# WangWen-Believer/DR-SLAM

Measured on AMD Instinct MI355X. Metric: RGB-D frames/sec (extract+match) at 640x480, higher is better.
Workload: dtype u8; 1 GPU; 640x480 synthetic RGB-D (TUM3 intrinsics), ORB extract 1000/1.2/8/20/7 + SearchByProjection(frame k, frame k-1, th=15) on consecutive frames; BASELINE config 2; batch_per_gpu=512, batches_in_flight_per_gpu=3, distinct_resident_input_batches_per_gpu=3, sequence_frames_per_rank=64

## Files before the change

dr_slam_amd/csrc/capi_match.cpp:

```cpp
#include "drfe_internal.h"
#include "match_internal.h"
#include "stage_layout.h"
#include "../../include/drfe_math.h"

#include <algorithm>
#include <cmath>
#include <cstdlib>
#include <cstring>
#include <new>
#include <thread>

template <class T>
static hipError_t dalloc(T** p, size_t n)
{
    *p = nullptr;
    return hipMalloc((void**)p, std::max<size_t>(n, 1) * sizeof(T));
}

void drfe_match_buffers_free(drfe_ctx* c)
{
    MatchBuffers* m = c->mb;
    if (!m) return;
    void* ptrs[] = {m->d_pairs, m->d_queries, m->d_mps, m->d_scale, m->d_candIdx, m->d_candKey, m->d_candCnt, m->d_candBest,
                    m->d_hist, m->d_initObs, m->d_bfIdx, m->d_bfDist, m->d_bfQ, m->d_bfT};
// ... 305 lines not shown
{
    if (!c || !offsets || slot < 0 || slot >= c->lastBatch || !c->glueValid) return c ? DRFE_ERR_STATE : DRFE_ERR_INVALID;
    int rc = drfe_stream_sync(c);
    if (rc != DRFE_OK) return rc;
    HIPCHK(c, hipMemcpy(offsets, c->d_gridOff + (size_t)slot * (DRFE_GRID_CELLS + 1), sizeof(int) * (DRFE_GRID_CELLS + 1),
                        hipMemcpyDeviceToHost));
    const int n = offsets[DRFE_GRID_CELLS];
    if (n > cap) return DRFE_ERR_CAPACITY;
    if (n && indices) HIPCHK(c, hipMemcpy(indices, c->d_gridIdx + (size_t)slot * c->maxKp, sizeof(int) * n, hipMemcpyDeviceToHost));
    return DRFE_OK;
}

}

int drfe_match_consecutive_stage(drfe_ctx* c, const float* Tcw, const float* Twc, const drfe_camera* cam, int mono, int nframes, hipStream_t s)
{
    MatchBuffers* m = drfe_match_buffers(c);
    if (!m) return DRFE_ERR_HIP;
    const int np = nframes - 1;
    const size_t pairBytes = sizeof(MatchPair) * (size_t)c->cfg.max_batch, poseBytes = sizeof(float) * 16 * (size_t)c->cfg.max_batch;
    if (!m->h_stage[0]) {
        m->stageBytes = pairBytes + poseBytes;
        for (int k = 0; k < 2; k++) {
            HIPCHK(c, hipHostMalloc(&m->h_stage[k], m->stageBytes, hipHostMallocDefault));
            HIPCHK(c, hipEventCreateWithFlags(&m->stageEv[k], hipEventDisableTiming));
            HIPCHK(c, hipEventRecord(m->stageEv[k], s));
        }
    }
    const int slotK = m->stageNext;
    m->stageNext ^= 1;
    HIPCHK(c, hipEventSynchronize(m->stageEv[slotK]));
    MatchPair* pairs = static_cast<MatchPair*>(m->h_stage[slotK]);
    float* poses = reinterpret_cast<float*>(static_cast<uint8_t*>(m->h_stage[slotK]) + pairBytes);
    std::memcpy(poses, Twc, sizeof(float) * 16 * (size_t)nframes);
    const float mb = cam->bf / cam->fx;
    for (int p = 0; p < np; p++) {
        MatchPair& P = pairs[p];
        P.curSlot = p + 1; P.lastSlot = p; P.mpSlot = p; P.nQueries = 0;
        P.queryBase = p * c->maxKp;
        P.mpBase = p * c->maxKp;
        std::memcpy(P.Tcw, Tcw + (size_t)(p + 1) * 16, sizeof(float) * 16);
        drfe_motion_flags(Tcw + (size_t)(p + 1) * 16, Tcw + (size_t)p * 16, mb, mono, &P.forward, &P.backward);
    }
    HIPCHK(c, hipMemcpyAsync(m->d_pairs, pairs, sizeof(MatchPair) * np, hipMemcpyHostToDevice, s));
    HIPCHK(c, hipMemcpyAsync(c->d_poses, poses, sizeof(float) * 16 * nframes, hipMemcpyHostToDevice, s));
    HIPCHK(c, hipEventRecord(m->stageEv[slotK], s));
    return DRFE_OK;
}

hipError_t drfe_match_consecutive_enqueue(drfe_ctx* c, const drfe_camera* cam, float th, int check_ori, int nframes, hipStream_t s)
{
    MatchBuffers* m = drfe_match_buffers(c);
    if (!m) return hipErrorOutOfMemory;
    hipError_t e = hipMemsetAsync(c->d_match, 0xFF, sizeof(int) * (size_t)nframes * c->maxKp, s);
    if (e == hipSuccess) e = hipMemsetAsync(c->d_matchCount, 0, sizeof(int) * nframes, s);
    if (e == hipSuccess) e = drfe_launch_mappoints_last(c, *m, *cam, c->d_poses, nframes, s);
    if (e == hipSuccess) e = drfe_launch_window_match(c, *m, *cam, nframes - 1, c->maxKp, 0, th, 0.f, check_ori, nullptr, s, 2);
    return e;
}

extern "C" {

int drfe_match_consecutive_batch(drfe_ctx* c, const float* Tcw, const float* Twc, const drfe_camera* cam, float th,
                                 int mono, int check_ori, int nframes, void* stream)
{
    if (!c || !Tcw || !Twc || !cam) return DRFE_ERR_INVALID;
    if (nframes < 2 || nframes > c->lastBatch || !c->glueValid) {
        c->err = "match: needs an extracted batch of >= 2 frames with stereo/grid computed";
        return DRFE_ERR_STATE;
    }
    if (c->maxKp > DRFE_MATCH_LAST_MAX_QUERIES) {
        c->err = "match: the slot size (drfe_orb_max_keypoints = " + std::to_string(c->maxKp) +
                 ") exceeds the 4096 map points the consecutive matcher resolves per pair";
        return DRFE_ERR_CAPACITY;
    }
    HIPCHK(c, hipSetDevice(c->device));
    hipStream_t s = stream ? (hipStream_t)stream : c->stream;
    const int rc = drfe_match_consecutive_stage(c, Tcw, Twc, cam, mono, nframes, s);
    if (rc != DRFE_OK) return rc;
    if (c->profile) { (void)hipEventRecord(c->ev[DRFE_STAGE_MATCH][0], s); c->evUsed[DRFE_STAGE_MATCH] = true; }
    HIPCHK(c, drfe_match_consecutive_enqueue(c, cam, th, check_ori, nframes, s));
    if (c->profile) (void)hipEventRecord(c->ev[DRFE_STAGE_MATCH][1], s);
    return DRFE_OK;
}

int drfe_match_download(drfe_ctx* c, int slot, int32_t* cur_to_last, int cap, int* nmatches)
{
    if (!c || slot < 0 || slot >= c->lastBatch) return c ? DRFE_ERR_STATE : DRFE_ERR_INVALID;
    int rc = drfe_stream_sync(c);
    if (rc != DRFE_OK) return rc;
    rc = match_status(c, 2);
    if (rc != DRFE_OK) return rc;
    int n = 0;
    HIPCHK(c, hipMemcpy(&n, c->d_kpCount + slot, sizeof(int), hipMemcpyDeviceToHost));
    if (n > cap) return DRFE_ERR_CAPACITY;
    if (n && cur_to_last)
        HIPCHK(c, hipMemcpy(cur_to_last, c->d_match + (size_t)slot * c->maxKp, sizeof(int) * n, hipMemcpyDeviceToHost));
    if (nmatches) HIPCHK(c, hipMemcpy(nmatches, c->d_matchCount + slot, sizeof(int), hipMemcpyDeviceToHost));
    return DRFE_OK;
}

int drfe_search_by_projection_last(drfe_ctx* c, int cur_slot, int last_slot, const float* Tcw_cur, const float* Tcw_last,
                                   const drfe_camera* cam, const drfe_map_point* last_mp, int n_last, float th, int mono,
                                   int check_ori, const uint8_t* cur_obs, int32_t* cur_mp, int n_cur, int* nmatches)
{
    if (!c || !Tcw_cur || !Tcw_last || !cam || !last_mp || !cur_mp || !nmatches) return DRFE_ERR_INVALID;
    if (cur_slot < 0 || cur_slot >= c->lastBatch || last_slot < 0 || last_slot >= c->lastBatch || !c->glueValid) {
        c->err = "search_by_projection_last: slots not ready";
        return DRFE_ERR_STATE;
    }
    HIPCHK(c, hipSetDevice(c->device));
// ... 854 lines not shown
```

dr_slam_amd/csrc/match_internal.h:

```cpp
#ifndef DRFE_MATCH_INTERNAL_H
#define DRFE_MATCH_INTERNAL_H
#include "drfe_internal.h"

#define DRFE_MATCH_LAST_MAX_QUERIES 4096

struct MatchPair {
    int curSlot, lastSlot;
    int mpSlot;
    int nQueries;
    int queryBase;
    int mpBase;
    int forward, backward;
    float Tcw[16];
};

struct MatchQuery {
    float u, v, radius;
    float ur, thrR;
    int minLevel, maxLevel;
    int valid;
    int obs;
    uint32_t desc[8];
};

struct MatchBuffers {
    MatchPair* d_pairs = nullptr;
    MatchQuery* d_queries = nullptr;
    drfe_map_point* d_mps = nullptr;
    float* d_scale = nullptr;
    uint32_t* d_candIdx = nullptr;
    uint32_t* d_candKey = nullptr;
    int* d_candCnt = nullptr;
    uint2* d_candBest = nullptr;
    uint16_t* d_hist = nullptr;
    uint8_t* d_initObs = nullptr;
    int32_t* d_bfIdx = nullptr; int32_t* d_bfDist = nullptr; uint8_t* d_bfQ = nullptr; uint8_t* d_bfT = nullptr; size_t bfCap = 0;
    size_t queryCap = 0;
    void* h_stage[2] = {nullptr, nullptr}; hipEvent_t stageEv[2] = {nullptr, nullptr}; size_t stageBytes = 0; int stageNext = 0;
};

hipError_t drfe_launch_window_match(drfe_ctx* c, const MatchBuffers& mb, const drfe_camera& cam, int npairs,
                                    int maxQueries, int mode, float th, float nnratio, int checkOri,
                                    const uint8_t* d_initObs, hipStream_t s, int statusWord = 1);
hipError_t drfe_launch_fill_i32(int* d_p, int n, int v, hipStream_t s);
hipError_t drfe_launch_fill_i32_and_word(int* d_p, int n, int v, int* d_q, int w, hipStream_t s);
struct DrfePackArgs { const uint32_t* src[10]; uint32_t dwords[10]; int n; };
hipError_t drfe_launch_pack_segments(const DrfePackArgs& A, uint32_t* d_dst, hipStream_t s);
void drfe_motion_flags(const float* TcwCur, const float* TcwLast, float mb, int mono, int* fwd, int* bwd);
hipError_t drfe_launch_window_candidates(drfe_ctx* c, const MatchBuffers& mb, const drfe_camera& cam, int npairs, int maxQueries,
                                         hipStream_t s);
hipError_t drfe_launch_mappoints_last(drfe_ctx* c, const MatchBuffers& mb, const drfe_camera& cam, const float* d_Twc,
                                      int nframes, hipStream_t s);
hipError_t drfe_launch_bf_knn(const uint8_t* dQ, int nq, const uint8_t* dT, int nt, int k, int* dIdx, int* dDist,
                              hipStream_t s);

struct LineQuery {
    int valid, obs;
    int minLevel, maxLevel;
    float x1, y1, x2, y2, r;
    uint32_t desc[8];
};
struct LineCur { float ptX, ptY, angle; int octave; };

hipError_t drfe_launch_line_projection(const drfe_map_line* d_lines, int n, const float* d_TcwCur, const drfe_camera& cam,
                                       int forward, int backward, const float* d_scale, float th, LineQuery* d_q,
                                       hipStream_t s);
hipError_t drfe_launch_line_search(const LineQuery* d_q, int n, const LineCur* d_cur, const uint8_t* d_desc, int nCur,
                                   float nnratio, uint8_t* d_claim, int* d_curMl, int* d_nmatches, hipStream_t s);

struct FrustumPose { float T[16]; float Ow[3]; float bf; float logScale; int nLevels; float limit; };
hipError_t drfe_launch_frustum_points(const drfe_frustum_point* d_pts, int n, const FrustumPose& P, const drfe_camera& cam,
                                      drfe_tracked_point* d_out, hipStream_t s);
hipError_t drfe_launch_frustum_lines(const drfe_frustum_line* d_lines, int n, const FrustumPose& P, const drfe_camera& cam,
                                     drfe_tracked_line* d_out, hipStream_t s);

struct LineSim3 { float sR[9], t[3]; };
hipError_t drfe_launch_line_fuse_search(const drfe_frustum_line* d_lines, const uint8_t* d_descs, const uint8_t* d_skip, int n,
                                        const FrustumPose& P, const drfe_camera& cam, const float* d_scale, float th,
                                        const LineCur* d_kf, const uint8_t* d_kfDesc, int nKF, int* d_bestIdx, int* d_bestDist,
                                        hipStream_t s, const LineSim3* sim3 = nullptr, int* d_distRow = nullptr);

struct FuseParams { float T[16]; float Ow[3]; float bf, logScale, th; int nLevels; float scale[16], invSigma2[16];
                    int sim3;
                    float sR2[9], t2[3];
                    int listTh; };
#define FUSE_LIST_K 8
hipError_t drfe_launch_fuse_search(drfe_ctx* c, int slot, const drfe_frustum_point* d_pts, const uint8_t* d_descs,
                                   const uint8_t* d_skip, int n, const FuseParams& P, const drfe_camera& cam, int* d_bestIdx,
                                   int* d_bestDist, hipStream_t s, const uint8_t* d_taken = nullptr, int2* d_list = nullptr,
                                   int* d_listCount = nullptr);

MatchBuffers* drfe_match_buffers(drfe_ctx* c);
int drfe_match_consecutive_stage(drfe_ctx* c, const float* Tcw, const float* Twc, const drfe_camera* cam, int mono, int nframes, hipStream_t s);
hipError_t drfe_match_consecutive_enqueue(drfe_ctx* c, const drfe_camera* cam, float th, int check_ori, int nframes, hipStream_t s);
void drfe_match_buffers_free(drfe_ctx* c);
#endif
```

dr_slam_amd/csrc/match_kernels.hip:

```cpp
#include "drfe_internal.h"
#include "match_internal.h"
#include "../../include/drfe_math.h"

#define WAVE 64


__global__ __launch_bounds__(256) void k_undistort(const drfe_keypoint* __restrict__ kps, const int* __restrict__ kpCount,
                                                   int maxKp, DrfeDistortion D, drfe_keypoint* __restrict__ kpsUn)
{
    const int slot = blockIdx.y;
    const int i = blockIdx.x * 256 + threadIdx.x;
    if (i >= kpCount[slot]) return;
    drfe_keypoint kp = kps[(size_t)slot * maxKp + i];
    float ux, uy;
    drfe_undistort_point(D, kp.x, kp.y, &ux, &uy);
    kp.x = ux; kp.y = uy;
    kpsUn[(size_t)slot * maxKp + i] = kp;
}

__global__ __launch_bounds__(256) void k_stereo(const drfe_keypoint* __restrict__ kps, const drfe_keypoint* __restrict__ kpsUn,
                                                const int* __restrict__ kpCount,
                                                int maxKp, const uint16_t* __restrict__ depth, size_t frameStride,
                                                size_t rowStride, int w, int h, drfe_camera cam,
                                                float* __restrict__ uRight, float* __restrict__ zDepth)
// ... 124 lines not shown
        p[1] = (kp.y - cam.cy) * z * invfy;
        p[2] = z;
        mat3_mul_add(Twc + (size_t)slot * 16, p, mp.world);
    }
    const uint32_t* d = reinterpret_cast<const uint32_t*>(desc + o * 32);
    uint32_t* md = reinterpret_cast<uint32_t*>(mp.desc);
#pragma unroll
    for (int k = 0; k < 8; k++) md[k] = d[k];
    mps[o] = mp;
}

__global__ __launch_bounds__(256) void k_queries_last(const MatchPair* __restrict__ pairs,
                                                      const drfe_keypoint* __restrict__ kps,
                                                      const int* __restrict__ kpCount, int maxKp,
                                                      const drfe_map_point* __restrict__ mps, drfe_camera cam,
                                                      const float* __restrict__ scaleFactors, float th,
                                                      MatchQuery* __restrict__ queries)
{
    const MatchPair P = pairs[blockIdx.y];
    const int i = blockIdx.x * 256 + threadIdx.x;
    const int nLast = P.mpSlot >= 0 ? kpCount[P.lastSlot] : P.nQueries;
    if (i >= nLast) return;
    MatchQuery q;
    q.valid = 0;
    q.u = q.v = q.radius = q.ur = q.thrR = 0.f;
    q.minLevel = q.maxLevel = -1;
    q.obs = 0;
    const drfe_map_point mp = mps[(size_t)P.mpBase + i];
#pragma unroll
    for (int k = 0; k < 8; k++) q.desc[k] = reinterpret_cast<const uint32_t*>(mp.desc)[k];
    q.obs = mp.obs_positive;
    if (mp.valid) {
        float xc[3];
        mat3_mul_add(P.Tcw, mp.world, xc);
        const float invzc = (float)(1.0 / (double)xc[2]);
        if (!(invzc < 0)) {
            const float u = cam.fx * xc[0] * invzc + cam.cx;
            const float v = cam.fy * xc[1] * invzc + cam.cy;
            if (!(u < cam.min_x || u > cam.max_x) && !(v < cam.min_y || v > cam.max_y)) {
                const int oct = kps[(size_t)P.lastSlot * maxKp + i].octave;
                const float radius = th * scaleFactors[oct];
                q.u = u; q.v = v; q.radius = radius; q.thrR = radius;
                q.ur = u - cam.bf * invzc;
                if (P.forward) { q.minLevel = oct; q.maxLevel = -1; }
                else if (P.backward) { q.minLevel = 0; q.maxLevel = oct; }
                else { q.minLevel = oct - 1; q.maxLevel = oct + 1; }
                q.valid = 1;
            }
        }
    }
    queries[(size_t)P.queryBase + i] = q;
}


__device__ __forceinline__ bool window_cells(const MatchQuery& q, const drfe_camera& cam, float invW, float invH, int& minX,
                                             int& maxX, int& minY, int& maxY)
{
    const float x = q.u, y = q.v, r = q.radius;
    minX = max(0, (int)floorf((x - cam.min_x - r) * invW));
    maxX = min(DRFE_GRID_COLS - 1, (int)ceilf((x - cam.min_x + r) * invW));
    minY = max(0, (int)floorf((y - cam.min_y - r) * invH));
    maxY = min(DRFE_GRID_ROWS - 1, (int)ceilf((y - cam.min_y + r) * invH));
    return !(minX >= DRFE_GRID_COLS || maxX < 0 || minY >= DRFE_GRID_ROWS || maxY < 0);
}

__device__ __forceinline__ bool window_candidate(const MatchQuery& q, bool bCheckLevels, const uint4* __restrict__ cK,
                                                 const uint4* __restrict__ cD, int p, int sq, uint64_t q0, uint64_t q1,
                                                 uint64_t q2, uint64_t q3, uint32_t& key, uint32_t& id)
{
    const uint4 k4 = cK[p];
    const uint4 da = cD[2 * p], db = cD[2 * p + 1];
    const float kx = __uint_as_float(k4.x), ky = __uint_as_float(k4.y), ur = __uint_as_float(k4.z);
    const int oct = (int)(k4.w >> 24);
    bool ok = true;
    if (bCheckLevels) {
        if (oct < q.minLevel) ok = false;
        if (q.maxLevel >= 0 && oct > q.maxLevel) ok = false;
    }
    const float dx = kx - q.u, dy = ky - q.v;
    if (!(fabsf(dx) < q.radius && fabsf(dy) < q.radius)) ok = false;
    if (ur > 0) {
        const float er = fabsf(q.ur - ur);
        if (er > q.thrR) ok = false;
    }
    if (!ok) return false;
    const int dist = __popcll(q0 ^ ((uint64_t)da.x | ((uint64_t)da.y << 32))) + __popcll(q1 ^ ((uint64_t)da.z | ((uint64_t)da.w << 32))) +
                     __popcll(q2 ^ ((uint64_t)db.x | ((uint64_t)db.y << 32))) + __popcll(q3 ^ ((uint64_t)db.z | ((uint64_t)db.w << 32)));
    key = ((uint32_t)dist << 22) | (uint32_t)min(sq, (1 << 22) - 1);
    id = k4.w;
    return true;
}

__device__ void window_query_wave(const MatchQuery& q, size_t qo, int lane, int nMinCellX, int nMaxCellX, int nMinCellY, int nMaxCellY,
                                  const int* __restrict__ gOff, const uint4* __restrict__ cK, const uint4* __restrict__ cD,
                                  uint32_t* __restrict__ candIdx, uint32_t* __restrict__ candKey, int* __restrict__ candCnt,
                                  uint2* __restrict__ candBest, int* __restrict__ status)
{
    const bool bCheckLevels = (q.minLevel > 0) || (q.maxLevel >= 0);
    uint32_t* oIdx = candIdx + qo * DRFE_MATCH_MAX_CAND;
    uint32_t* oKey = candKey + qo * DRFE_MATCH_MAX_CAND;
    const uint64_t q0 = (uint64_t)q.desc[0] | ((uint64_t)q.desc[1] << 32), q1 = (uint64_t)q.desc[2] | ((uint64_t)q.desc[3] << 32),
                   q2 = (uint64_t)q.desc[4] | ((uint64_t)q.desc[5] << 32), q3 = (uint64_t)q.desc[6] | ((uint64_t)q.desc[7] << 32);
    const int ncol = nMaxCellX - nMinCellX + 1;
    int runB = 0, runN = 0;
    if (lane < ncol) {
        const int cb = (nMinCellX + lane) * DRFE_GRID_ROWS;
        runB = gOff[cb + nMinCellY];
        runN = gOff[cb + nMaxCellY + 1] - runB;
    }
    const int incl = drfe_wave_incl_scan(runN, lane);
    const int T = __builtin_amdgcn_readlane(incl, 63);
    int nOut = 0;
    bool overflow = false;
    uint32_t myKey = 0xFFFFFFFFu, myIdx = 0;
    for (int s0 = 0; s0 < T; s0 += WAVE) {
        const int sq = s0 + lane;
        bool pass = false;
        uint32_t key = 0xFFFFFFFFu, id = 0;
        int base = __builtin_amdgcn_readfirstlane(runB);
        for (int j = 0; j + 1 < ncol; j++) {
            const int inclJ = __builtin_amdgcn_readlane(incl, j), nextB = __builtin_amdgcn_readlane(runB, j + 1);
            if (inclJ <= sq) base = nextB - inclJ;
        }
        if (sq < T) pass = window_candidate(q, bCheckLevels, cK, cD, base + sq, sq, q0, q1, q2, q3, key, id);
        const unsigned long long m = __ballot(pass);
        const int pos = nOut + __popcll(m & ((1ull << lane) - 1ull));
        if (pass) {
            if (pos < DRFE_MATCH_MAX_CAND) {
                oIdx[pos] = id;
                oKey[pos] = key;
                if (key < myKey) { myKey = key; myIdx = id; }
            } else overflow = true;
        }
        nOut += __popcll(m);
    }
    if (__any(overflow) && lane == 0) atomicOr(status, 4);
    const uint32_t mn = drfe_wave_min_u32(myKey);
    const unsigned long long who = __ballot(myKey == mn);
    const uint32_t bIdx = (uint32_t)__builtin_amdgcn_readlane((int)myIdx, __ffsll((long long)who) - 1);
    if (lane == 0) {
        candCnt[qo] = min(nOut, DRFE_MATCH_MAX_CAND);
        candBest[qo] = make_uint2(mn, bIdx);
    }
}

#define WQ_TAB 64
#ifndef WQ_THREADS
#define WQ_THREADS 64
#endif
#define WQ_PER_BLOCK (WQ_THREADS / WAVE * 4)
__global__ __launch_bounds__(WQ_THREADS) void k_window_candidates(const MatchPair* __restrict__ pairs,
                                                           const MatchQuery* __restrict__ queries,
                                                           const int* __restrict__ kpCount, int maxKp,
                                                           const int* __restrict__ gridOff,
                                                           const uint4* __restrict__ cellKp,
                                                           const uint4* __restrict__ cellDesc, drfe_camera cam,
                                                           float invW, float invH,
                                                           uint32_t* __restrict__ candIdx,
                                                           uint32_t* __restrict__ candKey,
                                                           int* __restrict__ candCnt, uint2* __restrict__ candBest,
                                                           int* __restrict__ status, uint32_t gxMagic)
{
    __shared__ int sTab[WQ_THREADS / WAVE][4][WQ_TAB];
    int bx, by;
    drfe_xcd_swizzle_2d(gxMagic, bx, by);
    const MatchPair P = pairs[by];
    const int wv = __builtin_amdgcn_readfirstlane((int)(threadIdx.x >> 6)), lane = threadIdx.x & 63;
    const int g = lane >> 4, l = lane & 15;
    const int qbase = (bx * (WQ_THREADS / WAVE) + wv) * 4;
    const int nQ = P.mpSlot >= 0 ? kpCount[P.lastSlot] : P.nQueries;
    if (qbase >= nQ) return;
    const int cur = P.curSlot;
    const int* gOff = gridOff + (size_t)cur * (DRFE_GRID_CELLS + 1);
    const uint4* cK = cellKp + (size_t)cur * maxKp;
    const uint4* cD = cellDesc + (size_t)cur * maxKp * 2;
    const bool have = qbase + g < nQ;
    const size_t qo = (size_t)P.queryBase + (have ? qbase + g : qbase);
    const MatchQuery q = queries[qo];
    int nMinCellX = 0, nMaxCellX = 0, nMinCellY = 0, nMaxCellY = 0;
    const bool inRange = have && q.valid && window_cells(q, cam, invW, invH, nMinCellX, nMaxCellX, nMinCellY, nMaxCellY);
    const int ncol = nMaxCellX - nMinCellX + 1;
    int runB = 0, runN = 0;
    const bool narrow = inRange && ncol <= 16;
    if (narrow && l < ncol) {
        const int cb = (nMinCellX + l) * DRFE_GRID_ROWS;
        runB = gOff[cb + nMinCellY];
        runN = gOff[cb + nMaxCellY + 1] - runB;
    }
    int incl = runN;
    incl += __builtin_amdgcn_update_dpp(0, incl, 0x111, 0xf, 0xf, true);
    incl += __builtin_amdgcn_update_dpp(0, incl, 0x112, 0xf, 0xf, true);
    incl += __builtin_amdgcn_update_dpp(0, incl, 0x114, 0xf, 0xf, true);
    incl += __builtin_amdgcn_update_dpp(0, incl, 0x118, 0xf, 0xf, true);
    const int T = __shfl(incl, 15, 16);
    const bool small = narrow && T <= WQ_TAB;
    {
        const int excl = incl - runN;
        const int n = small ? runN : 0;
        for (int k = 0; __any(k < n); k++)
            if (k < n) sTab[wv][g][excl + k] = runB + k;
    }
    const bool bCheckLevels = (q.minLevel > 0) || (q.maxLevel >= 0);
    const uint64_t q0 = (uint64_t)q.desc[0] | ((uint64_t)q.desc[1] << 32), q1 = (uint64_t)q.desc[2] | ((uint64_t)q.desc[3] << 32),
                   q2 = (uint64_t)q.desc[4] | ((uint64_t)q.desc[5] << 32), q3 = (uint64_t)q.desc[6] | ((uint64_t)q.desc[7] << 32);
    uint32_t* oIdx = candIdx + qo * DRFE_MATCH_MAX_CAND;
    uint32_t* oKey = candKey + qo * DRFE_MATCH_MAX_CAND;
    const int Tg = small ? T : 0;
    int nOut = 0;
    uint32_t myKey = 0xFFFFFFFFu, myIdx = 0;
    for (int s0 = 0; __any(s0 < Tg); s0 += 16) {
        const int sq = s0 + l;
        bool pass = false;
        uint32_t key = 0xFFFFFFFFu, id = 0;
        if (sq < Tg) pass = window_candidate(q, bCheckLevels, cK, cD, sTab[wv][g][sq], sq, q0, q1, q2, q3, key, id);
        const uint32_t m16 = (uint32_t)(__ballot(pass) >> (g * 16)) & 0xFFFFu;
        const int pos = nOut + __popc(m16 & ((1u << l) - 1u));
        if (pass) {
            oIdx[pos] = id;
            oKey[pos] = key;
            if (key < myKey) { myKey = key; myIdx = id; }
        }
        nOut += __popc(m16);
    }
    uint32_t mn = myKey;
    mn = min(mn, (uint32_t)__builtin_amdgcn_update_dpp((int)mn, (int)mn, 0xB1, 0xf, 0xf, false));
    mn = min(mn, (uint32_t)__builtin_amdgcn_update_dpp((int)mn, (int)mn, 0x4E, 0xf, 0xf, false));
    mn = min(mn, (uint32_t)__builtin_amdgcn_update_dpp((int)mn, (int)mn, 0x141, 0xf, 0xf, false));
    mn = min(mn, (uint32_t)__builtin_amdgcn_update_dpp((int)mn, (int)mn, 0x140, 0xf, 0xf, false));
    const uint32_t who16 = (uint32_t)(__ballot(myKey == mn) >> (g * 16)) & 0xFFFFu;
    const uint32_t bIdx = (uint32_t)__shfl((int)myIdx, __ffs((int)who16) - 1, 16);
    if (have && l == 0 && (small || !inRange)) {
        candCnt[qo] = nOut;
        candBest[qo] = small ? make_uint2(mn, bIdx) : make_uint2(0xFFFFFFFFu, 0u);
    }
    unsigned long long wide = __ballot(inRange && !small && l == 0);
    while (wide) {
        const int gg = (__ffsll((long long)wide) - 1) >> 4;
        wide &= wide - 1;
        const size_t qw = (size_t)P.queryBase + qbase + gg;
        const MatchQuery qq = queries[qw];
        int x0, x1, y0, y1;
        window_cells(qq, cam, invW, invH, x0, x1, y0, y1);
        window_query_wave(qq, qw, lane, x0, x1, y0, y1, gOff, cK, cD, candIdx, candKey, candCnt, candBest, status);
    }
}


__device__ __forceinline__ uint32_t wave_min_u32(uint32_t v) { return drfe_wave_min_u32(v); }

#define RS_THREADS 512
#define RS_MAX_T 8
static_assert(RS_THREADS * RS_MAX_T == DRFE_MATCH_LAST_MAX_QUERIES, "the C-ABI checks this limit before launching");
__global__ __launch_bounds__(RS_THREADS) void k_resolve_last(const MatchPair* __restrict__ pairs,
                                                             const MatchQuery* __restrict__ queries,
                                                             const drfe_keypoint* __restrict__ kps,
                                                             const int* __restrict__ kpCount, int maxKp,
                                                             const uint32_t* __restrict__ candIdx,
                                                             const uint32_t* __restrict__ candKey,
                                                             const int* __restrict__ candCnt,
                                                             const uint2* __restrict__ candBest, int checkOri,
                                                             int* __restrict__ match ,
                                                             const uint8_t* __restrict__ initObs,
                                                             int* __restrict__ matchCount,
                                                             uint16_t* __restrict__ histScratch )
{
    extern __shared__ int rs_smem[];
    int* owner = rs_smem;
    unsigned char* claim = reinterpret_cast<unsigned char*>(rs_smem + maxKp);
    __shared__ int hist[30];
    __shared__ int sNm, sEnt, sInd[3], sChanged[3];
    const MatchPair P = pairs[blockIdx.x];
    const int tid = threadIdx.x;
    const int nQ = P.mpSlot >= 0 ? kpCount[P.lastSlot] : P.nQueries;
    const int nCur = kpCount[P.curSlot];
    int* M = match + (size_t)P.curSlot * maxKp;
    const drfe_keypoint* Kc = kps + (size_t)P.curSlot * maxKp;
    const drfe_keypoint* Kl = kps + (size_t)P.lastSlot * maxKp;
    uint16_t* hs = histScratch + (size_t)blockIdx.x * 2 * maxKp;
    for (int i = tid; i < nCur; i += RS_THREADS) {
        unsigned char c = 0;
        if (M[i] >= 0) c = 1 | ((initObs ? initObs[i] : 1) ? 2 : 0);
        claim[i] = c;
    }
    if (tid < 30) hist[tid] = 0;
    if (tid == 0) { sNm = 0; sEnt = 0; sChanged[0] = 0; }
    const float factor = 1.0f / 30;
    int cnt[RS_MAX_T], obs[RS_MAX_T];
    uint32_t bKey[RS_MAX_T], bIdx[RS_MAX_T], pKey[RS_MAX_T], pIdx[RS_MAX_T];
#pragma unroll
    for (int t = 0; t < RS_MAX_T; t++) {
        const int i = tid + t * RS_THREADS;
        cnt[t] = 0; obs[t] = 0; bKey[t] = 0xFFFFFFFFu; bIdx[t] = 0; pKey[t] = 0xFFFFFFFFu; pIdx[t] = 0;
        if (i < nQ) {
            const size_t qo = (size_t)P.queryBase + i;
            cnt[t] = candCnt[qo];
            if (cnt[t] > 0) { const uint2 b = candBest[qo]; bKey[t] = b.x; bIdx[t] = b.y; obs[t] = queries[qo].obs; }
        }
    }
    for (int sweep = 0;; sweep++) {
        for (int k = tid; k < nCur; k += RS_THREADS) owner[k] = 0x7FFFFFFF;
        if (tid == 0) sChanged[(sweep + 1) % 3] = 0;
        __syncthreads();
#pragma unroll
        for (int t = 0; t < RS_MAX_T; t++)
            if (obs[t] && pKey[t] != 0xFFFFFFFFu && (int)(pKey[t] >> 22) <= 100)
                atomicMin(&owner[pIdx[t] & 0xFFFFFF], tid + t * RS_THREADS);
        __syncthreads();
        bool changed = false;
#pragma unroll
        for (int t = 0; t < RS_MAX_T; t++) {
            if (cnt[t] == 0) continue;
            const int i = tid + t * RS_THREADS;
            uint32_t key = 0xFFFFFFFFu, idx = 0;
            const int kb = (int)(bIdx[t] & 0xFFFFFF);
            if ((claim[kb] & 3) != 3 && owner[kb] >= i) { key = bKey[t]; idx = bIdx[t]; }
            else {
                const size_t qo = ((size_t)P.queryBase + i) * DRFE_MATCH_MAX_CAND;
                for (int j0 = 0; j0 < cnt[t]; j0 += 8) {
                    const uint4 ka = *reinterpret_cast<const uint4*>(candKey + qo + j0);
                    const uint4 kb2 = *reinterpret_cast<const uint4*>(candKey + qo + j0 + 4);
                    const uint4 ia = *reinterpret_cast<const uint4*>(candIdx + qo + j0);
                    const uint4 ib = *reinterpret_cast<const uint4*>(candIdx + qo + j0 + 4);
                    const uint32_t kv[8] = {ka.x, ka.y, ka.z, ka.w, kb2.x, kb2.y, kb2.z, kb2.w};
                    const uint32_t iv[8] = {ia.x, ia.y, ia.z, ia.w, ib.x, ib.y, ib.z, ib.w};
#pragma unroll
                    for (int u = 0; u < 8; u++) {
                        if (j0 + u >= cnt[t] || kv[u] >= key) continue;
                        const int kk = (int)(iv[u] & 0xFFFFFF);
                        if ((claim[kk] & 3) != 3 && owner[kk] >= i) { key = kv[u]; idx = iv[u]; }
                    }
                }
            }
            if (key != pKey[t] || idx != pIdx[t]) { changed = true; pKey[t] = key; pIdx[t] = idx; }
        }
        if (changed) sChanged[sweep % 3] = 1;
        __syncthreads();
        if (!__builtin_amdgcn_readfirstlane(sChanged[sweep % 3])) break;
    }
    for (int k = tid; k < nCur; k += RS_THREADS) owner[k] = -1;
    __syncthreads();
#pragma unroll
    for (int t = 0; t < RS_MAX_T; t++) {
        if (pKey[t] == 0xFFFFFFFFu || (int)(pKey[t] >> 22) > 100) continue;
        const int i = tid + t * RS_THREADS;
        const int i2 = (int)(pIdx[t] & 0xFFFFFF);
        atomicMax(&owner[i2], i);
        atomicAdd(&sNm, 1);
        if (checkOri) {
            float rot = Kl[i].angle - Kc[i2].angle;
            if (rot < 0.0f) rot += 360.0f;
            int bin = (int)roundf(rot * factor);
            if (bin == 30) bin = 0;
            const int e = atomicAdd(&sEnt, 1);
            hs[2 * e] = (uint16_t)bin;
            hs[2 * e + 1] = (uint16_t)i2;
            atomicAdd(&hist[bin], 1);
        }
    }
    __syncthreads();
    for (int k = tid; k < nCur; k += RS_THREADS)
        if (owner[k] >= 0) M[k] = owner[k];
    __syncthreads();
    if (checkOri) {
        if (tid == 0) {
            int max1 = 0, max2 = 0, max3 = 0, ind1 = -1, ind2 = -1, ind3 = -1;
            for (int i = 0; i < 30; i++) {
                const int s = hist[i];
                if (s > max1) { max3 = max2; max2 = max1; max1 = s; ind3 = ind2; ind2 = ind1; ind1 = i; }
                else if (s > max2) { max3 = max2; max2 = s; ind3 = ind2; ind2 = i; }
                else if (s > max3) { max3 = s; ind3 = i; }
            }
            if (max2 < 0.1f * (float)max1) { ind2 = -1; ind3 = -1; }
            else if (max3 < 0.1f * (float)max1) { ind3 = -1; }
            sInd[0] = ind1; sInd[1] = ind2; sInd[2] = ind3;
        }
        __syncthreads();
        const int nEnt = sEnt;
        for (int e = tid; e < nEnt; e += RS_THREADS) {
            const int bin = hs[2 * e];
            if (bin != sInd[0] && bin != sInd[1] && bin != sInd[2]) { M[hs[2 * e + 1]] = -1; atomicSub(&sNm, 1); }
        }
        __syncthreads();
    }
    if (tid == 0) matchCount[P.curSlot] = sNm;
}

__global__ __launch_bounds__(WAVE) void k_resolve_map(const MatchPair* __restrict__ pairs,
                                                      const MatchQuery* __restrict__ queries,
                                                      const int* __restrict__ kpCount, int maxKp,
                                                      const uint32_t* __restrict__ candIdx,
                                                      const uint32_t* __restrict__ candKey,
                                                      const int* __restrict__ candCnt, float nnratio,
                                                      int* __restrict__ match, const uint8_t* __restrict__ initObs,
                                                      int* __restrict__ matchCount)
{
    extern __shared__ unsigned char claim[];
    const MatchPair P = pairs[blockIdx.x];
    const int lane = threadIdx.x;
    const int nQ = P.nQueries;
    const int nCur = kpCount[P.curSlot];
    int* M = match + (size_t)P.curSlot * maxKp;
    for (int i = lane; i < nCur; i += WAVE) {
        unsigned char c = 0;
        if (M[i] >= 0) c = 1 | ((initObs ? initObs[i] : 1) ? 2 : 0);
        claim[i] = c;
    }
    __syncthreads();
    int nmatches = 0;
    for (int i = 0; i < nQ; i++) {
        const size_t qo = (size_t)P.queryBase + i;
        const int cnt = candCnt[qo];
        if (cnt == 0) continue;
        uint32_t k1 = 0xFFFFFFFFu, i1 = 0, k2 = 0xFFFFFFFFu, i2 = 0;
        for (int c0 = 0; c0 < cnt; c0 += WAVE) {
// ... 125 lines not shown
    if (i < n) p[i] = v;
}
hipError_t drfe_launch_fill_i32(int* d_p, int n, int v, hipStream_t s)
{
    if (n <= 0) return hipSuccess;
    hipLaunchKernelGGL(k_fill_i32, dim3((n + 255) / 256), dim3(256), 0, s, d_p, n, v);
    return hipGetLastError();
}

__global__ __launch_bounds__(256) void k_fill_i32_and_word(int* __restrict__ p, int n, int v, int* __restrict__ q, int w)
{
    const int i = blockIdx.x * 256 + threadIdx.x;
    if (i < n) p[i] = v;
    if (i == 0) *q = w;
}
hipError_t drfe_launch_fill_i32_and_word(int* d_p, int n, int v, int* d_q, int w, hipStream_t s)
{
    hipLaunchKernelGGL(k_fill_i32_and_word, dim3((n > 0 ? n + 255 : 256) / 256), dim3(256), 0, s, d_p, n, v, d_q, w);
    return hipGetLastError();
}

__global__ __launch_bounds__(256) void k_pack_segments(DrfePackArgs A, uint32_t* __restrict__ dst)
{
    uint32_t total = 0;
    for (int k = 0; k < A.n; k++) total += A.dwords[k];
    for (uint32_t i = blockIdx.x * 256 + threadIdx.x; i < total; i += gridDim.x * 256) {
        uint32_t base = 0;
        int k = 0;
        while (i - base >= A.dwords[k]) { base += A.dwords[k]; k++; }
        if (A.src[k]) dst[i] = A.src[k][i - base];
    }
}
hipError_t drfe_launch_pack_segments(const DrfePackArgs& A, uint32_t* d_dst, hipStream_t s)
{
    uint32_t total = 0;
    for (int k = 0; k < A.n; k++) total += A.dwords[k];
    if (!total) return hipSuccess;
    const unsigned blocks = (total + 1023) / 1024;
    hipLaunchKernelGGL(k_pack_segments, dim3(blocks), dim3(256), 0, s, A, d_dst);
    return hipGetLastError();
}

hipError_t drfe_launch_window_match(drfe_ctx* c, const MatchBuffers& mb, const drfe_camera& cam, int npairs,
                                    int maxQueries, int mode, float th, float nnratio, int checkOri,
                                    const uint8_t* d_initObs, hipStream_t s, int statusWord)
{
    const float invW = (float)DRFE_GRID_COLS / (float)(cam.max_x - cam.min_x);
    const float invH = (float)DRFE_GRID_ROWS / (float)(cam.max_y - cam.min_y);
    if (mode == 0 && maxQueries > RS_THREADS * RS_MAX_T) return hipErrorInvalidValue;
    (void)drfe_launch_fill_i32(c->d_status + statusWord, 1, 0, s);
    if (mode == 0)
        hipLaunchKernelGGL(k_queries_last, dim3((maxQueries + 255) / 256, npairs), dim3(256), 0, s, mb.d_pairs,
                           drfe_kps_un(c), c->d_kpCount, c->maxKp, mb.d_mps, cam, mb.d_scale, th, mb.d_queries);
    hipLaunchKernelGGL(k_window_candidates, dim3((maxQueries + WQ_PER_BLOCK - 1) / WQ_PER_BLOCK, npairs), dim3(WQ_THREADS), 0, s, mb.d_pairs,
                       mb.d_queries, c->d_kpCount, c->maxKp, c->d_gridOff, c->d_cellKp, c->d_cellDesc, cam, invW, invH,
                       mb.d_candIdx, mb.d_candKey, mb.d_candCnt, mb.d_candBest, c->d_status + statusWord,
                       drfe_div_magic((uint32_t)((maxQueries + WQ_PER_BLOCK - 1) / WQ_PER_BLOCK)));
    const size_t lds = (size_t)c->maxKp;
    if (mode == 0)
        hipLaunchKernelGGL(k_resolve_last, dim3(npairs), dim3(RS_THREADS), (size_t)c->maxKp * 5 + 16, s, mb.d_pairs,
                           mb.d_queries, drfe_kps_un(c), c->d_kpCount, c->maxKp, mb.d_candIdx, mb.d_candKey, mb.d_candCnt,
                           mb.d_candBest, checkOri, c->d_match, d_initObs, c->d_matchCount, mb.d_hist);
    else
        hipLaunchKernelGGL(k_resolve_map, dim3(npairs), dim3(WAVE), lds, s, mb.d_pairs, mb.d_queries, c->d_kpCount,
                           c->maxKp, mb.d_candIdx, mb.d_candKey, mb.d_candCnt, nnratio, c->d_match, d_initObs,
                           c->d_matchCount);
    return hipGetLastError();
}

hipError_t drfe_launch_window_candidates(drfe_ctx* c, const MatchBuffers& mb, const drfe_camera& cam, int npairs, int maxQueries,
                                         hipStream_t s)
{
    const float invW = (float)DRFE_GRID_COLS / (float)(cam.max_x - cam.min_x);
    const float invH = (float)DRFE_GRID_ROWS / (float)(cam.max_y - cam.min_y);
    (void)hipMemsetAsync(c->d_status + 1, 0, sizeof(int), s);
    hipLaunchKernelGGL(k_window_candidates, dim3((maxQueries + WQ_PER_BLOCK - 1) / WQ_PER_BLOCK, npairs), dim3(WQ_THREADS), 0, s, mb.d_pairs,
                       mb.d_queries, c->d_kpCount, c->maxKp, c->d_gridOff, c->d_cellKp, c->d_cellDesc, cam, invW, invH,
                       mb.d_candIdx, mb.d_candKey, mb.d_candCnt, mb.d_candBest, c->d_status + 1,
                       drfe_div_magic((uint32_t)((maxQueries + WQ_PER_BLOCK - 1) / WQ_PER_BLOCK)));
    return hipGetLastError();
}

hipError_t drfe_launch_mappoints_last(drfe_ctx* c, const MatchBuffers& mb, const drfe_camera& cam, const float* d_Twc,
                                      int nframes, hipStream_t s)
{
    hipLaunchKernelGGL(k_mappoints_last, dim3((c->maxKp + 255) / 256, nframes), dim3(256), 0, s, drfe_kps_un(c), c->d_desc,
                       c->d_kpCount, c->maxKp, c->d_depth, cam, d_Twc, mb.d_mps);
    return hipGetLastError();
}

hipError_t drfe_launch_bf_knn(const uint8_t* dQ, int nq, const uint8_t* dT, int nt, int k, int* dIdx, int* dDist,
                              hipStream_t s)
{
    hipLaunchKernelGGL(k_bf_knn, dim3((nq + 63) / 64), dim3(64), 0, s, dQ, nq, dT, nt, k, dIdx, dDist);
    return hipGetLastError();
}


__global__ __launch_bounds__(64) void k_line_queries_last(const drfe_map_line* __restrict__ lines, int n,
                                                          const float* __restrict__ TcwCur, drfe_camera cam, int forward,
                                                          int backward, const float* __restrict__ scale, float th,
                                                          LineQuery* __restrict__ out)
{
    const int i = blockIdx.x * 64 + threadIdx.x;
    if (i >= n) return;
    const drfe_map_line ml = lines[i];
    LineQuery q;
    q.valid = 0; q.obs = ml.obs_positive ? 1 : 0; q.minLevel = 0; q.maxLevel = 0;
    q.x1 = q.y1 = q.x2 = q.y2 = q.r = 0.f;
#pragma unroll
    for (int k = 0; k < 8; k++) q.desc[k] = reinterpret_cast<const uint32_t*>(ml.desc)[k];
    if (ml.valid) {
        const float SP[3] = {(float)ml.world[0], (float)ml.world[1], (float)ml.world[2]};
        const float EP[3] = {(float)ml.world[3], (float)ml.world[4], (float)ml.world[5]};
        float T[16];
#pragma unroll
        for (int k = 0; k < 16; k++) T[k] = TcwCur[k];
        float SPc[3], EPc[3];
        mat3_mul_add(T, SP, SPc);
        mat3_mul_add(T, EP, EPc);
        bool ok = !(SPc[2] < 0.0f || EPc[2] < 0.0f);
        const float invz1 = 1.0f / SPc[2];
        const float u1 = cam.fx * SPc[0] * invz1 + cam.cx, v1 = cam.fy * SPc[1] * invz1 + cam.cy;
        if (u1 < cam.min_x || u1 > cam.max_x || v1 < cam.min_y || v1 > cam.max_y) ok = false;
        const float invz2 = 1.0f / EPc[2];
        const float u2 = cam.fx * EPc[0] * invz2 + cam.cx, v2 = cam.fy * EPc[1] * invz2 + cam.cy;
        if (u2 < cam.min_x || u2 > cam.max_x || v2 < cam.min_y || v2 > cam.max_y) ok = false;
        if (ok) {
            const int oct = ml.octave;
            q.valid = 1;
            q.x1 = u1; q.y1 = v1; q.x2 = u2; q.y2 = v2;
            q.r = th * scale[oct];
// ... 424 lines not shown
```

Before: 282,200 frames/s.

## Fuse consecutive-frame matching into compact query pipeline without memsets and map-point pass

Replaces the consecutive matcher's memsets, map-point construction kernel and full query build with a compact query kernel. That kernel back-projects depth and reprojects in one step and writes 32-byte records, with descriptors read directly from the last frame. The resolve kernel gains a batch specialization that skips the claim initialization and writes every match slot itself, so the separate d_match/matchCount memsets are no longer needed. This cuts launches, global traffic and intermediate map-point writes, at the cost of template duplication and reuse of the d_queries buffer with a different record layout.

New measurement: 283,900 frames/s (median of 6 runs). About the same (+0.6%).

```diff
diff --git a/dr_slam_amd/csrc/capi_match.cpp b/dr_slam_amd/csrc/capi_match.cpp
--- a/dr_slam_amd/csrc/capi_match.cpp
+++ b/dr_slam_amd/csrc/capi_match.cpp
@@ -381,11 +381,7 @@
 {
     MatchBuffers* m = drfe_match_buffers(c);
     if (!m) return hipErrorOutOfMemory;
-    hipError_t e = hipMemsetAsync(c->d_match, 0xFF, sizeof(int) * (size_t)nframes * c->maxKp, s);
-    if (e == hipSuccess) e = hipMemsetAsync(c->d_matchCount, 0, sizeof(int) * nframes, s);
-    if (e == hipSuccess) e = drfe_launch_mappoints_last(c, *m, *cam, c->d_poses, nframes, s);
-    if (e == hipSuccess) e = drfe_launch_window_match(c, *m, *cam, nframes - 1, c->maxKp, 0, th, 0.f, check_ori, nullptr, s, 2);
-    return e;
+    return drfe_launch_match_consecutive_kernels(c, *m, *cam, c->d_poses, nframes, th, check_ori, s);
 }
 
 extern "C" {
diff --git a/dr_slam_amd/csrc/match_internal.h b/dr_slam_amd/csrc/match_internal.h
--- a/dr_slam_amd/csrc/match_internal.h
+++ b/dr_slam_amd/csrc/match_internal.h
@@ -22,6 +22,15 @@
     int obs;
     uint32_t desc[8];
 };
+
+struct alignas(16) MatchQueryCompact {
+    float u, v, radius, ur;
+    int minLevel, maxLevel;
+    int valid;
+    int pad;
+};
+static_assert(sizeof(MatchQueryCompact) == 32 && sizeof(MatchQueryCompact) <= sizeof(MatchQuery),
+              "the compact records live in the d_queries block");
 
 struct MatchBuffers {
     MatchPair* d_pairs = nullptr;
@@ -49,6 +58,8 @@
 void drfe_motion_flags(const float* TcwCur, const float* TcwLast, float mb, int mono, int* fwd, int* bwd);
 hipError_t drfe_launch_window_candidates(drfe_ctx* c, const MatchBuffers& mb, const drfe_camera& cam, int npairs, int maxQueries,
                                          hipStream_t s);
+hipError_t drfe_launch_match_consecutive_kernels(drfe_ctx* c, const MatchBuffers& mb, const drfe_camera& cam, const float* d_Twc,
+                                                 int nframes, float th, int checkOri, hipStream_t s);
 hipError_t drfe_launch_mappoints_last(drfe_ctx* c, const MatchBuffers& mb, const drfe_camera& cam, const float* d_Twc,
                                       int nframes, hipStream_t s);
 hipError_t drfe_launch_bf_knn(const uint8_t* dQ, int nq, const uint8_t* dT, int nt, int k, int* dIdx, int* dDist,
diff --git a/dr_slam_amd/csrc/match_kernels.hip b/dr_slam_amd/csrc/match_kernels.hip
--- a/dr_slam_amd/csrc/match_kernels.hip
+++ b/dr_slam_amd/csrc/match_kernels.hip
@@ -200,6 +200,54 @@
     queries[(size_t)P.queryBase + i] = q;
 }
 
+__global__ __launch_bounds__(256) void k_queries_consecutive(const MatchPair* __restrict__ pairs,
+                                                             const drfe_keypoint* __restrict__ kps,
+                                                             const int* __restrict__ kpCount, int maxKp,
+                                                             const float* __restrict__ zDepth, drfe_camera cam,
+                                                             const float* __restrict__ Twc ,
+                                                             const float* __restrict__ scaleFactors, float th,
+                                                             MatchQueryCompact* __restrict__ queries,
+                                                             int* __restrict__ status)
+{
+    const MatchPair P = pairs[blockIdx.y];
+    const int i = blockIdx.x * 256 + threadIdx.x;
+    if (i == 0 && blockIdx.y == 0) *status = 0;
+    if (i >= kpCount[P.lastSlot]) return;
+    const size_t o = (size_t)P.lastSlot * maxKp + i;
+    MatchQueryCompact q;
+    q.valid = 0;
+    q.u = q.v = q.radius = q.ur = 0.f;
+    q.minLevel = q.maxLevel = -1;
+    q.pad = 0;
+    const float z = zDepth[o];
+    if (z > 0) {
+        const float invfx = 1.0f / cam.fx, invfy = 1.0f / cam.fy;
+        const drfe_keypoint kp = kps[o];
+        float p[3], world[3], xc[3];
+        p[0] = (kp.x - cam.cx) * z * invfx;
+        p[1] = (kp.y - cam.cy) * z * invfy;
+        p[2] = z;
+        mat3_mul_add(Twc + (size_t)P.lastSlot * 16, p, world);
+        mat3_mul_add(P.Tcw, world, xc);
+        const float invzc = (float)(1.0 / (double)xc[2]);
+        if (!(invzc < 0)) {
+            const float u = cam.fx * xc[0] * invzc + cam.cx;
+            const float v = cam.fy * xc[1] * invzc + cam.cy;
+            if (!(u < cam.min_x || u > cam.max_x) && !(v < cam.min_y || v > cam.max_y)) {
+                const int oct = kp.octave;
+                const float radius = th * scaleFactors[oct];
+                q.u = u; q.v = v; q.radius = radius;
+                q.ur = u - cam.bf * invzc;
+                if (P.forward) { q.minLevel = oct; q.maxLevel = -1; }
+                else if (P.backward) { q.minLevel = 0; q.maxLevel = oct; }
+                else { q.minLevel = oct - 1; q.maxLevel = oct + 1; }
+                q.valid = 1;
+            }
+        }
+    }
+    queries[(size_t)P.queryBase + i] = q;
+}
+
 
 __device__ __forceinline__ bool window_cells(const MatchQuery& q, const drfe_camera& cam, float invW, float invH, int& minX,
                                              int& maxX, int& minY, int& maxY)
@@ -297,8 +345,30 @@
 #define WQ_THREADS 64
 #endif
 #define WQ_PER_BLOCK (WQ_THREADS / WAVE * 4)
+template <bool COMPACT>
+__device__ __forceinline__ MatchQuery window_load_query(const void* __restrict__ queries, const MatchPair& P, int i,
+                                                        const uint8_t* __restrict__ desc, int maxKp)
+{
+    if constexpr (!COMPACT) return static_cast<const MatchQuery*>(queries)[(size_t)P.queryBase + i];
+    else {
+        const uint4* r = reinterpret_cast<const uint4*>(static_cast<const MatchQueryCompact*>(queries) + ((size_t)P.queryBase + i));
+        const uint4* d = reinterpret_cast<const uint4*>(desc + ((size_t)P.lastSlot * maxKp + i) * 32);
+        const uint4 a = r[0], b = r[1], da = d[0], db = d[1];
+        MatchQuery q;
+        q.u = __uint_as_float(a.x); q.v = __uint_as_float(a.y); q.radius = __uint_as_float(a.z); q.ur = __uint_as_float(a.w);
+        q.thrR = q.radius;
+        q.minLevel = (int)b.x; q.maxLevel = (int)b.y; q.valid = (int)b.z;
+        q.obs = 1;
+        q.desc[0] = da.x; q.desc[1] = da.y; q.desc[2] = da.z; q.desc[3] = da.w;
+        q.desc[4] = db.x; q.desc[5] = db.y; q.desc[6] = db.z; q.desc[7] = db.w;
+        return q;
+    }
+}
+
+template <bool COMPACT>
 __global__ __launch_bounds__(WQ_THREADS) void k_window_candidates(const MatchPair* __restrict__ pairs,
-                                                           const MatchQuery* __restrict__ queries,
+                                                           const void* __restrict__ queries,
+                                                           const uint8_t* __restrict__ descLast,
                                                            const int* __restrict__ kpCount, int maxKp,
                                                            const int* __restrict__ gridOff,
                                                            const uint4* __restrict__ cellKp,
@@ -323,8 +393,9 @@
     const uint4* cK = cellKp + (size_t)cur * maxKp;
     const uint4* cD = cellDesc + (size_t)cur * maxKp * 2;
     const bool have = qbase + g < nQ;
-    const size_t qo = (size_t)P.queryBase + (have ? qbase + g : qbase);
-    const MatchQuery q = queries[qo];
+    const int qi = have ? qbase + g : qbase;
+    const size_t qo = (size_t)P.queryBase + qi;
+    const MatchQuery q = window_load_query<COMPACT>(queries, P, qi, descLast, maxKp);
     int nMinCellX = 0, nMaxCellX = 0, nMinCellY = 0, nMaxCellY = 0;
     const bool inRange = have && q.valid && window_cells(q, cam, invW, invH, nMinCellX, nMaxCellX, nMinCellY, nMaxCellY);
     const int ncol = nMaxCellX - nMinCellX + 1;
@@ -386,7 +457,7 @@
         const int gg = (__ffsll((long long)wide) - 1) >> 4;
         wide &= wide - 1;
         const size_t qw = (size_t)P.queryBase + qbase + gg;
-        const MatchQuery qq = queries[qw];
+        const MatchQuery qq = window_load_query<COMPACT>(queries, P, qbase + gg, descLast, maxKp);
         int x0, x1, y0, y1;
         window_cells(qq, cam, invW, invH, x0, x1, y0, y1);
         window_query_wave(qq, qw, lane, x0, x1, y0, y1, gOff, cK, cD, candIdx, candKey, candCnt, candBest, status);
@@ -399,6 +470,7 @@
 #define RS_THREADS 512
 #define RS_MAX_T 8
 static_assert(RS_THREADS * RS_MAX_T == DRFE_MATCH_LAST_MAX_QUERIES, "the C-ABI checks this limit before launching");
+template <bool BATCH>
 __global__ __launch_bounds__(RS_THREADS) void k_resolve_last(const MatchPair* __restrict__ pairs,
                                                              const MatchQuery* __restrict__ queries,
                                                              const drfe_keypoint* __restrict__ kps,
@@ -425,11 +497,12 @@
     const drfe_keypoint* Kc = kps + (size_t)P.curSlot * maxKp;
     const drfe_keypoint* Kl = kps + (size_t)P.lastSlot * maxKp;
     uint16_t* hs = histScratch + (size_t)blockIdx.x * 2 * maxKp;
-    for (int i = tid; i < nCur; i += RS_THREADS) {
-        unsigned char c = 0;
-        if (M[i] >= 0) c = 1 | ((initObs ? initObs[i] : 1) ? 2 : 0);
-        claim[i] = c;
-    }
+    if constexpr (!BATCH)
+        for (int i = tid; i < nCur; i += RS_THREADS) {
+            unsigned char c = 0;
+            if (M[i] >= 0) c = 1 | ((initObs ? initObs[i] : 1) ? 2 : 0);
+            claim[i] = c;
+        }
     if (tid < 30) hist[tid] = 0;
     if (tid == 0) { sNm = 0; sEnt = 0; sChanged[0] = 0; }
     const float factor = 1.0f / 30;
@@ -442,7 +515,7 @@
         if (i < nQ) {
             const size_t qo = (size_t)P.queryBase + i;
             cnt[t] = candCnt[qo];
-            if (cnt[t] > 0) { const uint2 b = candBest[qo]; bKey[t] = b.x; bIdx[t] = b.y; obs[t] = queries[qo].obs; }
+            if (cnt[t] > 0) { const uint2 b = candBest[qo]; bKey[t] = b.x; bIdx[t] = b.y; obs[t] = BATCH ? 1 : queries[qo].obs; }
         }
     }
     for (int sweep = 0;; sweep++) {
@@ -461,7 +534,7 @@
             const int i = tid + t * RS_THREADS;
             uint32_t key = 0xFFFFFFFFu, idx = 0;
             const int kb = (int)(bIdx[t] & 0xFFFFFF);
-            if ((claim[kb] & 3) != 3 && owner[kb] >= i) { key = bKey[t]; idx = bIdx[t]; }
+            if ((BATCH || (claim[kb] & 3) != 3) && owner[kb] >= i) { key = bKey[t]; idx = bIdx[t]; }
             else {
                 const size_t qo = ((size_t)P.queryBase + i) * DRFE_MATCH_MAX_CAND;
                 for (int j0 = 0; j0 < cnt[t]; j0 += 8) {
@@ -475,7 +548,7 @@
                     for (int u = 0; u < 8; u++) {
                         if (j0 + u >= cnt[t] || kv[u] >= key) continue;
                         const int kk = (int)(iv[u] & 0xFFFFFF);
-                        if ((claim[kk] & 3) != 3 && owner[kk] >= i) { key = kv[u]; idx = iv[u]; }
+                        if ((BATCH || (claim[kk] & 3) != 3) && owner[kk] >= i) { key = kv[u]; idx = iv[u]; }
                     }
                 }
             }
@@ -506,8 +579,15 @@
         }
     }
     __syncthreads();
-    for (int k = tid; k < nCur; k += RS_THREADS)
-        if (owner[k] >= 0) M[k] = owner[k];
+    if constexpr (BATCH) {
+        for (int k = tid; k < maxKp; k += RS_THREADS) M[k] = k < nCur ? owner[k] : -1;
+        if (blockIdx.x == 0) {
+            for (int k = tid; k < maxKp; k += RS_THREADS) match[k] = -1;
+            if (tid == 0) matchCount[0] = 0;
+        }
+    } else
+        for (int k = tid; k < nCur; k += RS_THREADS)
+            if (owner[k] >= 0) M[k] = owner[k];
     __syncthreads();
     if (checkOri) {
         if (tid == 0) {
@@ -739,13 +819,13 @@
     if (mode == 0)
         hipLaunchKernelGGL(k_queries_last, dim3((maxQueries + 255) / 256, npairs), dim3(256), 0, s, mb.d_pairs,
                            drfe_kps_un(c), c->d_kpCount, c->maxKp, mb.d_mps, cam, mb.d_scale, th, mb.d_queries);
-    hipLaunchKernelGGL(k_window_candidates, dim3((maxQueries + WQ_PER_BLOCK - 1) / WQ_PER_BLOCK, npairs), dim3(WQ_THREADS), 0, s, mb.d_pairs,
-                       mb.d_queries, c->d_kpCount, c->maxKp, c->d_gridOff, c->d_cellKp, c->d_cellDesc, cam, invW, invH,
+    hipLaunchKernelGGL(k_window_candidates<false>, dim3((maxQueries + WQ_PER_BLOCK - 1) / WQ_PER_BLOCK, npairs), dim3(WQ_THREADS), 0, s, mb.d_pairs,
+                       mb.d_queries, nullptr, c->d_kpCount, c->maxKp, c->d_gridOff, c->d_cellKp, c->d_cellDesc, cam, invW, invH,
                        mb.d_candIdx, mb.d_candKey, mb.d_candCnt, mb.d_candBest, c->d_status + statusWord,
                        drfe_div_magic((uint32_t)((maxQueries + WQ_PER_BLOCK - 1) / WQ_PER_BLOCK)));
     const size_t lds = (size_t)c->maxKp;
     if (mode == 0)
-        hipLaunchKernelGGL(k_resolve_last, dim3(npairs), dim3(RS_THREADS), (size_t)c->maxKp * 5 + 16, s, mb.d_pairs,
+        hipLaunchKernelGGL(k_resolve_last<false>, dim3(npairs), dim3(RS_THREADS), (size_t)c->maxKp * 5 + 16, s, mb.d_pairs,
                            mb.d_queries, drfe_kps_un(c), c->d_kpCount, c->maxKp, mb.d_candIdx, mb.d_candKey, mb.d_candCnt,
                            mb.d_candBest, checkOri, c->d_match, d_initObs, c->d_matchCount, mb.d_hist);
     else
@@ -761,10 +841,31 @@
     const float invW = (float)DRFE_GRID_COLS / (float)(cam.max_x - cam.min_x);
     const float invH = (float)DRFE_GRID_ROWS / (float)(cam.max_y - cam.min_y);
     (void)hipMemsetAsync(c->d_status + 1, 0, sizeof(int), s);
-    hipLaunchKernelGGL(k_window_candidates, dim3((maxQueries + WQ_PER_BLOCK - 1) / WQ_PER_BLOCK, npairs), dim3(WQ_THREADS), 0, s, mb.d_pairs,
-                       mb.d_queries, c->d_kpCount, c->maxKp, c->d_gridOff, c->d_cellKp, c->d_cellDesc, cam, invW, invH,
+    hipLaunchKernelGGL(k_window_candidates<false>, dim3((maxQueries + WQ_PER_BLOCK - 1) / WQ_PER_BLOCK, npairs), dim3(WQ_THREADS), 0, s, mb.d_pairs,
+                       mb.d_queries, nullptr, c->d_kpCount, c->maxKp, c->d_gridOff, c->d_cellKp, c->d_cellDesc, cam, invW, invH,
                        mb.d_candIdx, mb.d_candKey, mb.d_candCnt, mb.d_candBest, c->d_status + 1,
                        drfe_div_magic((uint32_t)((maxQueries + WQ_PER_BLOCK - 1) / WQ_PER_BLOCK)));
+    return hipGetLastError();
+}
+
+hipError_t drfe_launch_match_consecutive_kernels(drfe_ctx* c, const MatchBuffers& mb, const drfe_camera& cam, const float* d_Twc,
+                                                 int nframes, float th, int checkOri, hipStream_t s)
+{
+    const float invW = (float)DRFE_GRID_COLS / (float)(cam.max_x - cam.min_x);
+    const float invH = (float)DRFE_GRID_ROWS / (float)(cam.max_y - cam.min_y);
+    const int npairs = nframes - 1, maxQueries = c->maxKp;
+    if (npairs < 1 || maxQueries > RS_THREADS * RS_MAX_T) return hipErrorInvalidValue;
+    MatchQueryCompact* d_q = reinterpret_cast<MatchQueryCompact*>(mb.d_queries);
+    int* d_status = c->d_status + 2;
+    const unsigned gx = (unsigned)((maxQueries + WQ_PER_BLOCK - 1) / WQ_PER_BLOCK);
+    hipLaunchKernelGGL(k_queries_consecutive, dim3((maxQueries + 255) / 256, npairs), dim3(256), 0, s, mb.d_pairs, drfe_kps_un(c),
+                       c->d_kpCount, c->maxKp, c->d_depth, cam, d_Twc, mb.d_scale, th, d_q, d_status);
+    hipLaunchKernelGGL(k_window_candidates<true>, dim3(gx, npairs), dim3(WQ_THREADS), 0, s, mb.d_pairs, d_q, c->d_desc,
+                       c->d_kpCount, c->maxKp, c->d_gridOff, c->d_cellKp, c->d_cellDesc, cam, invW, invH, mb.d_candIdx,
+                       mb.d_candKey, mb.d_candCnt, mb.d_candBest, d_status, drfe_div_magic(gx));
+    hipLaunchKernelGGL(k_resolve_last<true>, dim3(npairs), dim3(RS_THREADS), (size_t)c->maxKp * 4, s, mb.d_pairs, nullptr,
+                       drfe_kps_un(c), c->d_kpCount, c->maxKp, mb.d_candIdx, mb.d_candKey, mb.d_candCnt, mb.d_candBest, checkOri,
+                       c->d_match, nullptr, c->d_matchCount, mb.d_hist);
     return hipGetLastError();
 }
 
```
